# morispi/CONSENT

Measured on AMD Instinct MI355X. Metric: corrected windows/sec, higher is better.
Workload: dtype u8/int16 (2-bit bases, integer DP); 1 GPU; pacbio_d150_msa150: synthetic PacBio-profile piles, 500 bp windows, depth 150, maxMSA 150, k=9, solid=4, commonKMers=8, minAnchors=2; distinct_windows_per_run=704512, engines_per_gpu=4, engines_requested=4, engine_allocation_runs=0, hw_queues=4, overflow_windows=0, template_fallback_windows=0

## Files before the change

### consent_amd/csrc/cw_index.h

```cpp
#ifndef CW_INDEX_H
#define CW_INDEX_H

#include "cw_device.h"

typedef __attribute__((address_space(3))) uint32_t* cw_l32w;
typedef __attribute__((address_space(3))) const uint32_t* cw_l32;
typedef __attribute__((address_space(1))) const uint32_t* cw_g32;
typedef __attribute__((address_space(3))) uint16_t* cw_l16w;
typedef __attribute__((address_space(1))) uint16_t* cw_g16w;
#define CW_IDX_THREADS 1024
#define CW_IDX_WAVES 16
#define CW_IDX_LDS_BYTES 163840
#define CW_TMAX 2048
#define CW_EX_SLOTS 1024
#define CW_EX_BITS 10
#define CW_EXP_SLOTS 8
#define CW_EXG_SLOTS 262144
#define CW_TH_SLOTS 4096
#ifndef CW_IDX_BYTES_MIN_N
#define CW_IDX_BYTES_MIN_N 64u
#endif
#define CW_IDX_STAGE_OFF 139776
#define CW_IDX_STAGE_N 192
#define CW_IDX_STAGE_WORDS ((CW_IDX_LDS_BYTES - CW_IDX_STAGE_OFF - 16 - CW_IDX_STAGE_N * 8) / 4)
// ... 635 lines not shown
    while (xe != 0ull && (uint32_t)(xe >> 32) != key + 1) { slot = (slot + 1) & (CW_EX_SLOTS - 1); xe = ex[slot]; }
    return (uint32_t)xe;
}
__device__ __forceinline__ uint32_t idx_nibble_cand(const uint32_t v, const uint32_t add) {
    return ((((v & 0x0F0F0F0Fu) + add) & 0x10101010u) >> 4) | (((((v >> 4) & 0x0F0F0F0Fu) + add) & 0x10101010u) >> 3);
}
__device__ __forceinline__ bool idx_export_walk(const IdxLds& L, const IdxWin& win, const DevScratch& sc, const cw_params& prm, const uint32_t n_keys, const uint32_t nib_words,
                                                const unsigned long long* exg, const bool big_ex, uint32_t& total, unsigned long long& _pt) {
    const int tid = threadIdx.x;
    const uint32_t* const tab = L.tab();
    const uint32_t keys_per_word = n_keys >= 8 ? 8 : n_keys;
    const uint32_t wpt = (nib_words + CW_IDX_THREADS - 1) / CW_IDX_THREADS;
    const uint32_t w_beg = min(nib_words, (uint32_t)tid * wpt), w_cnt = min(nib_words, w_beg + wpt) - w_beg;
    uint32_t lk[CW_EXP_SLOTS];
    bool wide = false;
    uint32_t mine = 0, n_first = 0xFFFFFFFFu;
    const uint32_t add = (16u - (prm.solid < 15u ? prm.solid : 15u)) * 0x01010101u;
    auto scan_word = [&](const uint32_t v, const uint32_t wd) {
        if (v == 0) return;
        uint32_t cand = idx_nibble_cand(v, add);
        if (keys_per_word < 8) cand &= (1u << (8 * ((keys_per_word + 1) / 2))) - 1u;
        while (cand) {
            const uint32_t bpos = (uint32_t)__ffs((int)cand) - 1u;
            cand &= cand - 1u;
            const uint32_t q = (bpos >> 3) * 2u + (bpos & 1u);
            const uint32_t nib = (v >> (4 * q)) & 15u;
            const uint32_t key = wd * 8 + q;
            uint32_t c = nib;
            if (nib == 15u) c = 15u + idx_ex_lookup(L.ex(), exg, big_ex, key);
            if (c < prm.solid) continue;
#pragma unroll
            for (int z = 0; z < CW_EXP_SLOTS; ++z) if ((uint32_t)z == mine) lk[z] = key | (c << 18);
            wide = wide || c >= (1u << 14);
            mine++;
        }
    };
    if (w_cnt && (w_cnt & 3u) == 0u) {
        const uint32_t nq = w_cnt >> 2, q0 = (uint32_t)tid % nq;
        for (uint32_t i = 0; i < nq; ++i) {
            uint32_t r = i + q0;
            if (r == nq) n_first = mine;
            r = r >= nq ? r - nq : r;
            const uint32_t wd = w_beg + 4u * r;
            const uint4 v4 = *(const uint4*)&tab[wd];
            if ((v4.x | v4.y | v4.z | v4.w) == 0u) continue;
            scan_word(v4.x, wd); scan_word(v4.y, wd + 1u); scan_word(v4.z, wd + 2u); scan_word(v4.w, wd + 3u);
        }
    } else {
        const uint32_t r0 = w_cnt ? (uint32_t)tid % w_cnt : 0u;
        for (uint32_t i = 0; i < w_cnt; ++i) {
            uint32_t r = i + r0;
            if (r == w_cnt) n_first = mine;
            r = r >= w_cnt ? r - w_cnt : r;
            scan_word(tab[w_beg + r], w_beg + r);
        }
    }
    CW_PROF(sc.ctr, CW_PS_IDX_EXPORT_SCAN, tid == 0);
    const uint32_t off = cw_block_exscan(mine, L.scan_tmp(), &total);
    const bool fits = total <= win.solid_cap;
    if (n_first > mine) n_first = mine;
    if (fits && (mine > CW_EXP_SLOTS || wide)) {
        CW_IDX_ROUTE(sc.ctr, true, CW_IR_REWALK);
        uint32_t o = win.solid_base + off;
        for (uint32_t i = 0; i < w_cnt && mine; ++i) {
            const uint32_t wd = w_beg + i;
            const uint32_t v = tab[wd];
            if (v == 0) continue;
            uint32_t cand = idx_nibble_cand(v, add);
            if (keys_per_word < 8) cand &= (1u << (8 * ((keys_per_word + 1) / 2))) - 1u;
            while (cand) {
                const uint32_t bpos = (uint32_t)__ffs((int)cand) - 1u;
                cand &= cand - 1u;
                const uint32_t q = (bpos >> 3) * 2u + (bpos & 1u);
                const uint32_t nib = (v >> (4 * q)) & 15u;
                const uint32_t key = wd * 8 + q;
                uint32_t c = nib;
                if (nib == 15u) c = 15u + idx_ex_lookup(L.ex(), exg, big_ex, key);
                if (c >= prm.solid) { sc.solid_key[o] = key; sc.solid_cnt[o] = c; o++; }
            }
        }
    } else if (fits && mine) {
#pragma unroll
        for (int z = 0; z < CW_EXP_SLOTS; ++z) {
            if ((uint32_t)z < mine) {
                const uint32_t pos = (uint32_t)z < n_first ? (uint32_t)z + (mine - n_first) : (uint32_t)z - n_first;
                sc.solid_key[win.solid_base + off + pos] = lk[z] & 0x3FFFFu;
                sc.solid_cnt[win.solid_base + off + pos] = lk[z] >> 18;
            }
        }
    }
    return fits;
}
__device__ __forceinline__ bool idx_export_nibbles(const IdxLds& L, const IdxWin& win, const DevScratch& sc, const cw_params& prm, const uint32_t n_keys, const uint32_t nib_words,
                                                   const bool big_ex, unsigned long long& _pt) {
    const int tid = threadIdx.x;
    const unsigned long long* const exg = idx_wg_scratch(sc);
    uint32_t total;
    bool fits;
    const uint32_t NI = nib_words >> 12;
    if (prm.solid <= 15u && (nib_words & 4095u) == 0u && NI >= 1u && NI <= 8u) {
        const uint32_t add = (16u - (prm.solid < 15u ? prm.solid : 15u)) * 0x01010101u;
        uint32_t m[8];
        CW_IDX_ROUTE(sc.ctr, tid == 0, CW_IR_EXPORT_MASKS);
        idx_read_masks<8>(L.tab(), NI, m, [&](const uint32_t v) -> uint32_t {
            const uint32_t c = idx_nibble_cand(v, add);
            return (c | (c >> 6) | (c >> 12) | (c >> 18)) & 0xFFu;
        });
        CW_PROF(sc.ctr, CW_PS_IDX_EXPORT_SCAN, tid == 0);
        fits = idx_export_masks<8>(m, L.tab(), NI, 0u, win.solid_base, L.scan_tmp(), sc.solid_key, sc.solid_cnt, total,
            [&](const uint32_t n) -> bool { return n <= win.solid_cap; },
            [&](const uint32_t v, const uint32_t q, const uint32_t key) -> uint32_t {
                uint32_t c = (v >> (4u * q)) & 15u;
                if (c == 15u) c += idx_ex_lookup(L.ex(), exg, big_ex, key);
                return c;
            });
    } else {
        CW_IDX_ROUTE(sc.ctr, tid == 0, CW_IR_EXPORT_WALK);
        fits = idx_export_walk(L, win, sc, prm, n_keys, nib_words, exg, big_ex, total, _pt);
    }
    if (tid == 0) {
        win.wi->n_solid = fits ? total : 0;
        if (!fits) idx_stop(win.wi, sc.ctr, CW_WHY_SOLIDCAP);
    }
    __syncthreads();
    return fits;
}

__device__ __forceinline__ void idx_template_table(const IdxLds& L, const IdxPile& pl, const IdxMatrix& M, const uint32_t k, const uint32_t nk0) {
    const int tid = threadIdx.x;
    uint32_t* const th = L.th(); uint32_t* const tkey = L.tkey();
    if (M.tfit) M.clear_lds(nk0 * M.Np);
    if (tid == 0) { L.misc()[4] = 0; L.misc()[5] = 0; }
    for (uint32_t i = tid; i < CW_TH_SLOTS; i += CW_IDX_THREADS) th[i] = 0;
    for (uint32_t i = tid; i < L.seen_words() * 32u; i += CW_IDX_THREADS) { L.tsup()[i] = 0; L.trep()[i] = 0; L.tcand()[i] = -1; }
    for (uint32_t tp = tid; tp < nk0; tp += CW_IDX_THREADS) tkey[tp] = pl.stw ? cw_kmer_at(pl.s_words, tp, k) : cw_kmer_at(pl.bases + pl.seq_word_off[pl.s0], tp, k);
    __syncthreads();
    for (uint32_t tp = tid; tp < nk0; tp += CW_IDX_THREADS) {
        const uint32_t key = tkey[tp];
        uint32_t bkt = CW_TH_HOME(key);
        for (bool placed = false; !placed; bkt = (bkt + 1) & (CW_TH_BUCKETS - 1)) {
            for (uint32_t j = 0; j < 4u && !placed; ++j) {
                const uint32_t prev = atomicCAS(&th[bkt * 4u + j], 0u, (tp + 1u) | CW_TH_FP(key));
                if (prev == 0) placed = true;
                else if ((prev & ~4095u) == CW_TH_FP(key) && tkey[CW_TH_POS(prev) - 1] == key) { L.trep()[CW_TH_POS(prev) - 1] = 1; placed = true; }
            }
        }
    }
    __syncthreads();
}

#define CW_IDX_HIT_CAP (CW_EXG_SLOTS * 2u)
__device__ __forceinline__ bool idx_hit_list(const IdxMatrix& M, const uint32_t N) { return !M.tfit && N <= 1024u; }

__device__ __forceinline__ void idx_support(const IdxLds& L, const IdxPile& pl, const IdxMatrix& M, const DevScratch& sc, const uint32_t k, const uint32_t kmask) {
    const int lane = threadIdx.x & 63, wave = threadIdx.x >> 6;
    const uint32_t N = pl.N, Np = M.Np;
    uint32_t* const th = L.th(); uint32_t* const tkey = L.tkey(); uint32_t* const tsup = L.tsup(); uint8_t* const trep = L.trep(); uint32_t* const misc = L.misc();
    uint16_t* const P_lds = M.P_lds;
    const bool tfit = M.tfit, hl = idx_hit_list(M, N);
    uint32_t* const hitlist = (uint32_t*)idx_wg_scratch(sc);
    const uint32_t hit_cap = CW_IDX_HIT_CAP;
    const bool fp_exact = k <= 10u;
    auto support_seq = [&](const auto words, const uint32_t len, const uint32_t s, uint32_t* my_seen) {
        const uint32_t nk = len >= k ? len - k + 1 : 0, nwd = (len + 15u) >> 4;
        for (uint32_t p0 = (uint32_t)lane * 4u; p0 < nk; p0 += 256u) {
            uint32_t key4[4], bkt4[4], e1[4];
            idx_keys4(idx_window(words, p0, nwd), k, kmask, key4);
#pragma unroll
            for (uint32_t q = 0; q < 4u; ++q) bkt4[q] = CW_TH_HOME(key4[q]);
            if (fp_exact) {
                auto match = [&](const uint4 v, const uint32_t fp1) -> uint32_t { return min(min(v.x - fp1, v.y - fp1), min(v.z - fp1, v.w - fp1)); };
                uint4 v4[4];
#pragma unroll
                for (uint32_t q = 0; q < 4u; ++q) v4[q] = p0 + q < nk ? *(const uint4*)&th[bkt4[q] * 4u] : make_uint4(0u, 0u, 0u, 0u);
                uint32_t pend = 0;
#pragma unroll
                for (uint32_t q = 0; q < 4u; ++q) { e1[q] = match(v4[q], CW_TH_FP(key4[q]) + 1u); if (e1[q] >= (uint32_t)CW_TMAX && v4[q].w != 0u) pend |= 1u << q; }
                while (__ballot(pend != 0u) != 0ull) {
#pragma unroll
                    for (uint32_t q = 0; q < 4u; ++q) {
                        if ((pend >> q) & 1u) {
                            bkt4[q] = (bkt4[q] + 1u) & (CW_TH_BUCKETS - 1);
                            const uint4 v = *(const uint4*)&th[bkt4[q] * 4u];
                            e1[q] = match(v, CW_TH_FP(key4[q]) + 1u);
                            if (e1[q] < (uint32_t)CW_TMAX || v.w == 0u) pend &= ~(1u << q);
                        }
                    }
                }
            } else {
#pragma unroll
                for (uint32_t q = 0; q < 4u; ++q) e1[q] = p0 + q < nk ? (uint32_t)cw_tpl_lookup(th, tkey, key4[q]) : 0xFFFFFFFFu;
            }
            uint32_t old4[4];
#pragma unroll
            for (uint32_t q = 0; q < 4u; ++q) {
                const uint32_t e = e1[q];
                old4[q] = e < (uint32_t)CW_TMAX ? atomicOr(&my_seen[e >> 5], 1u << (e & 31u)) : 0u;
            }
            uint32_t n_list = 0, my_list = 0;
#pragma unroll
            for (uint32_t q = 0; q < 4u; ++q) {
                const uint32_t e = e1[q], p = p0 + q;
                const bool hit = e < (uint32_t)CW_TMAX;
                if (hit) {
                    if (old4[q] & (1u << (e & 31u))) trep[e] = 1;
                    else atomicAdd(&tsup[e], 1u);
                    if (tfit) P_lds[__umul24(e, Np) + s] = (uint16_t)p;
                    else if (hl && p >= 2048u) misc[5] = 1;
                }
                if (!tfit && hl) {
                    const unsigned long long hm = __ballot(hit && p < 2048u);
                    if (hit && p < 2048u) my_list |= (n_list + (uint32_t)__popcll(hm & ((1ull << lane) - 1ull))) << (8u * q);
                    n_list += (uint32_t)__popcll(hm);
                }
            }
            if (!tfit && hl && n_list) {
                uint32_t base = 0;
                if (lane == 0) base = atomicAdd(&misc[4], n_list);
                base = (uint32_t)cw_lane_value((int)base, 0);
#pragma unroll
                for (uint32_t q = 0; q < 4u; ++q) {
                    const uint32_t p = p0 + q, hi_ = base + ((my_list >> (8u * q)) & 255u);
                    if (e1[q] < (uint32_t)CW_TMAX && p < 2048u && hi_ < hit_cap) hitlist[hi_] = (e1[q] << 21) | (s << 11) | p;
                }
            }
        }
    };
    for (uint32_t s = wave; s < N; s += CW_IDX_WAVES) {
        uint32_t* my_seen = L.seen() + wave * L.seen_words();
        if ((uint32_t)lane < L.seen_words()) my_seen[lane] = 0;
        cw_wave_sync();
        idx_with_seq(pl, s, [&](const auto words, const uint32_t len) { support_seq(words, len, s, my_seen); });
        cw_wave_sync();
    }
    __syncthreads();
}

__device__ __forceinline__ uint32_t idx_candidates(const IdxLds& L, const uint32_t nk0, const int sup_min) {
    const int tid = threadIdx.x;
    uint32_t A = 0;
    for (uint32_t tb = 0; tb < nk0; tb += CW_IDX_THREADS) {
        const uint32_t tp = tb + (uint32_t)tid;
        uint32_t ok = 0;
        if (tp < nk0) {
            const int rep = cw_tpl_lookup(L.th(), L.tkey(), L.tkey()[tp]);
            ok = (rep == (int)tp && L.trep()[tp] == 0 && (int)L.tsup()[tp] >= sup_min) ? 1u : 0u;
        }
        uint32_t a_round;
        const uint32_t off = A + cw_block_exscan(ok, L.scan_tmp(), &a_round);
        if (ok) { L.tcand()[tp] = (int16_t)off; L.cand_tp()[off] = (uint16_t)tp; }
        A += a_round;
        __syncthreads();
    }
    __syncthreads();
    return A;
}

__device__ __forceinline__ bool idx_fill_matrix(const IdxLds& L, const IdxPile& pl, const IdxWin& win, const IdxMatrix& M, const DevScratch& sc, const uint32_t k, const uint32_t kmask,
                                                const uint32_t A) {
    const int tid = threadIdx.x, wave = tid >> 6;
    const uint32_t N = pl.N, Np = M.Np;
    if (M.pg && (uint64_t)A * Np > sc.p_fallback_elems) {
        if (tid == 0) { idx_stop(win.wi, sc.ctr, CW_WHY_MATRIX); win.wi->arena_used = (uint64_t)A * Np > 0xFFFFFFFFull ? 0xFFFFFFFFu : A * Np; }
        __builtin_amdgcn_wave_barrier();
        return false;
    }
    const uint32_t* const hitlist = (const uint32_t*)idx_wg_scratch(sc);
    const uint32_t n_hits = L.misc()[4];
    const bool from_list = idx_hit_list(M, N) && n_hits <= CW_IDX_HIT_CAP && L.misc()[5] == 0u;
    if (!M.tfit) {
        if (!M.pg) M.clear_lds(A * Np);
        else for (uint32_t i = tid; i < A * Np; i += CW_IDX_THREADS) M.wr(i, CW_NONE16);
        __builtin_amdgcn_fence(__ATOMIC_RELEASE, "workgroup");
        __syncthreads();
        __builtin_amdgcn_fence(__ATOMIC_ACQUIRE, "workgroup");
        if (from_list) {
            for (uint32_t i0 = tid; i0 < n_hits; i0 += 4u * CW_IDX_THREADS) {
                uint32_t h4[4];
#pragma unroll
                for (uint32_t u = 0; u < 4u; ++u) { const uint32_t i = i0 + u * CW_IDX_THREADS; h4[u] = i < n_hits ? hitlist[i] : 0xFFFFFFFFu; }
#pragma unroll
                for (uint32_t u = 0; u < 4u; ++u) {
                    const uint32_t h = h4[u];
                    const int a = i0 + u * CW_IDX_THREADS < n_hits ? L.tcand()[h >> 21] : -1;
                    if (a >= 0) M.wr((uint32_t)a * Np + ((h >> 11) & 1023u), h & 2047u);
                }
            }
        } else
        for (uint32_t s = wave; s < N; s += CW_IDX_WAVES) {
            idx_pile_seq<IDX_WAVE>(pl, s, k, kmask, [&](const uint32_t, const uint32_t p, const uint32_t key, const uint32_t) {
                const int e = cw_tpl_lookup(L.th(), L.tkey(), key);
                if (e < 0) return;
                const int a = L.tcand()[e];
                if (a >= 0) M.wr((uint32_t)a * Np + s, p);
            });
        }
        __syncthreads();
    }
    return true;
}

struct IdxPres {
    uint8_t* clean;
    uint8_t* didx;
    unsigned long long* pres;
    uint16_t* dirty;
    unsigned long long* badm;
    uint8_t* rowid;
    uint16_t* rowanc;
    bool use_bits, has_bm, has_delta;
    uint32_t n_rows;
    uint32_t W;
    uint32_t n_dirty;
};
__device__ __forceinline__ IdxPres idx_presence_carve(const IdxLds& L, const IdxMatrix& M, const uint32_t A, const uint32_t N, const uint32_t nk0) {
    uint8_t* const lds = L.lds;
    const uint32_t Nw = (N + 63u) >> 6;
    IdxPres ps;
    ps.clean = (uint8_t*)L.seen();
    ps.didx = ps.clean + 1024;
    ps.pres = (unsigned long long*)(M.P_lds + (M.pg ? 0 : (((size_t)(M.tfit ? nk0 : A) * M.Np + 3u) & ~(size_t)3u)));
    ps.dirty = (uint16_t*)(ps.pres + (size_t)A * Nw);
    ps.badm = (unsigned long long*)(lds + (((size_t)((uint8_t*)(ps.dirty + N) - lds) + 7u) & ~(size_t)7u));
    ps.use_bits = N <= 2048u && ((uint8_t*)(ps.dirty + N) <= lds + CW_IDX_STAGE_OFF);
    ps.has_bm = false; ps.has_delta = false;
    ps.n_rows = 0;
    ps.W = 1;
    ps.rowid = (uint8_t*)(ps.badm + (size_t)A * 4);
    ps.rowanc = (uint16_t*)(lds + (((size_t)(ps.rowid + A - lds) + 1u) & ~(size_t)1u));
    ps.n_dirty = 0;
    return ps;
}

__device__ __forceinline__ IdxPres idx_classify_sequences(const IdxLds& L, const IdxWin& win, const IdxMatrix& M, IdxPres ps, const DevScratch& sc, const uint32_t A, unsigned long long& _pt) {
    const int tid = threadIdx.x, lane = tid & 63, wave = tid >> 6;
    const uint32_t N = win.N, Np = M.Np;
    uint8_t* const lds = L.lds; uint32_t* const misc = L.misc();
    uint8_t* const clean = ps.clean; uint16_t* const dirty = ps.dirty; unsigned long long* const badm = ps.badm;
    uint32_t W = 1;
    auto scan_seq = [&](const uint32_t s, const bool fwd, const bool mark, const uint32_t d) -> uint32_t {
        int run = -1;
        uint32_t n_bad = 0;
        for (uint32_t a0 = 0; a0 < A; a0 += 64) {
            const uint32_t ai = a0 + lane;
            const uint32_t a = fwd ? ai : A - 1u - ai;
            const uint32_t pv = ai < A ? M.rd(M.row(a) * Np + s) : (uint32_t)CW_NONE16;
            const int v = pv != CW_NONE16 ? (fwd ? (int)pv : (int)(0xFFFEu - pv)) : -1;
            const int inc = cw_wave_scan_max(v);
            int before = cw_wave_shr1(inc, -1);
            before = max(before, run);
            const bool bad = v >= 0 && v <= before;
            if (mark) { if (bad) atomicOr(&badm[(size_t)a * W + (d >> 6)], 1ull << (d & 63u)); }
            else n_bad += (uint32_t)__popcll(__ballot(bad));
            run = max(run, cw_lane_value(inc, 63));
        }
        return n_bad;
    };
    for (uint32_t s = wave; s < N; s += CW_IDX_WAVES) {
        const uint32_t nf = scan_seq(s, true, false, 0);
        uint32_t c = 1;
        if (nf) c = scan_seq(s, false, false, 0) < nf ? 2u : 0u;
        if (lane == 0) clean[s] = (uint8_t)c;
    }
    if (tid == 0) misc[3] = 0;
    __syncthreads();
    CW_PROF(sc.ctr, CW_PS_IDX_CLEAN, tid == 0);
    for (uint32_t s = tid; s < N; s += CW_IDX_THREADS)
        if (clean[s] != 1) dirty[atomicAdd(&misc[3], 1u)] = (uint16_t)s;
    __syncthreads();
    const uint32_t nd = misc[3];
    W = (nd + 63u) >> 6;
    if (W == 0u) W = 1u;
    const bool masks = nd > 0 && nd <= 255u  && W <= (N <= 1024u ? 4u : 1u) && (uint8_t*)(ps.rowanc + CW_AB_ROWS_MAX) <= lds + CW_IDX_STAGE_OFF;
    if (masks) {
        for (uint32_t i = tid; i < A * W; i += CW_IDX_THREADS) badm[i] = 0ull;
        __syncthreads();
        for (uint32_t d = wave; d < nd; d += CW_IDX_WAVES) { const uint32_t s = dirty[d]; scan_seq(s, clean[s] == 0, true, d); }
        __syncthreads();
        uint32_t ok2[2] = {0u, 0u}, off2[2] = {0u, 0u};
        uint32_t n_rows = 0;
#pragma nounroll
        for (uint32_t r2 = 0; r2 < 2u; ++r2) {
            const uint32_t an = r2 * CW_IDX_THREADS + (uint32_t)tid;
            if (r2 * CW_IDX_THREADS >= A) break;
            if (an < A) for (uint32_t x = 0; x < W; ++x) ok2[r2] |= badm[(size_t)an * W + x] != 0ull ? 1u : 0u;
            uint32_t n_round;
            off2[r2] = n_rows + cw_block_exscan(ok2[r2], misc + 16, &n_round);
            n_rows += n_round;
            __syncthreads();
        }
        ps.has_delta = n_rows >= 1u && n_rows <= CW_AB_ROWS_MAX && cw_ab_bytes(A, N, nd, n_rows) <= ((uint64_t)win.ab_cap << 4);
        ps.has_bm = W == 1u || ps.has_delta;
        if (ps.has_delta) {
            for (uint32_t r2 = 0; r2 < 2u; ++r2) {
                const uint32_t an = r2 * CW_IDX_THREADS + (uint32_t)tid;
                if (an < A) ps.rowid[an] = ok2[r2] ? (uint8_t)off2[r2] : (uint8_t)0xFF;
                if (ok2[r2]) ps.rowanc[off2[r2]] = (uint16_t)an;
            }
        } else n_rows = 0;
        ps.n_rows = n_rows;
        if (ps.has_bm && (uint32_t)tid < nd) { const uint32_t s = dirty[tid]; clean[s] = (uint8_t)0x80u; if (N <= 1024u) ps.didx[s] = (uint8_t)tid; else clean[s] = (uint8_t)(0x80u | (uint32_t)tid); }
        __syncthreads();
    }
    ps.W = W;
    return ps;
}

__device__ __forceinline__ void idx_presence(const IdxMatrix& M, const IdxPres& ps, const uint32_t A, const uint32_t N) {
    const int lane = threadIdx.x & 63, wave = threadIdx.x >> 6;
    const uint32_t Np = M.Np, Nw = (N + 63u) >> 6, W = ps.W;
    for (uint32_t w = 0; w < Nw; ++w) {
        const uint32_t s = w * 64 + lane;
        const uint32_t c = s < N ? (uint32_t)ps.clean[s] : 0u;
        const bool plain = c == 1u, part = ps.has_bm && (c & 0x80u) != 0u;
        const uint32_t d = part ? (N <= 1024u ? (uint32_t)ps.didx[s] : (c & 63u)) : 0u;
        for (uint32_t a = wave; a < A; a += CW_IDX_WAVES) {
            bool good = plain;
            if (part) good = !((ps.badm[(size_t)a * W + (d >> 6)] >> (d & 63u)) & 1ull);
            const bool on = s < N && M.rd(M.row(a) * Np + s) != CW_NONE16 && good;
            const unsigned long long bal = __ballot(on);
            if (lane == 0) ps.pres[(size_t)a * Nw + w] = bal;
        }
    }
    __syncthreads();
}

__device__ __forceinline__ bool idx_hand_over(const IdxLds& L, const IdxWin& win, const IdxMatrix& M, const IdxPres& ps, const DevScratch& sc, const uint32_t A) {
    const int tid = threadIdx.x, lane = tid & 63, wave = tid >> 6;
    const uint32_t N = win.N, Np = M.Np, Nw = (N + 63u) >> 6, W = ps.W, n_dirty = ps.n_dirty, n_rows = ps.n_rows;
    const unsigned long long* const badm = ps.badm; const uint16_t* const dirty = ps.dirty;
    if (cw_ab_bytes(A, N, n_dirty, n_rows) > ((uint64_t)win.ab_cap << 4)) {
        if (tid == 0) { idx_stop(win.wi, sc.ctr, CW_WHY_MATRIX); win.wi->arena_used = 0xFFFFFFFFu; }
        __builtin_amdgcn_wave_barrier();
        return false;
    }
    const CwAbCarve<uint8_t*> ab = cw_ab_carve(sc.ablock + ((size_t)win.ab_base << 4), A, N, n_dirty, n_rows);
    uint32_t* hdr = (uint32_t*)ab.hdr; uint32_t* ckey = (uint32_t*)ab.ckey; unsigned long long* gpres = (unsigned long long*)ab.pres; uint16_t* gdirty = (uint16_t*)ab.dirty;
    unsigned long long* gbadm = (unsigned long long*)ab.badm;
    const uint32_t Ap = cw_ab_ap(A);
    if (tid == 0) { hdr[0] = A; hdr[1] = N; hdr[2] = n_dirty; hdr[3] = (ps.use_bits ? 1u : 0u) | (ps.has_bm && W == 1u ? 2u : 0u) | (ps.has_delta ? 4u : 0u); hdr[4] = n_rows; }
    for (uint32_t a = tid; a < A; a += CW_IDX_THREADS) ckey[a] = L.tkey()[L.cand_tp()[a]];
    if (ps.use_bits) {
        for (uint32_t i = tid; i < A * Nw; i += CW_IDX_THREADS) gpres[i] = ps.pres[i];
        for (uint32_t i = tid; i < n_dirty; i += CW_IDX_THREADS) gdirty[i] = dirty[i];
        if (ps.has_bm && W == 1u) for (uint32_t a = tid; a < A; a += CW_IDX_THREADS) gbadm[a] = badm[a];
        if (ps.has_delta) {
            for (uint32_t a = tid; a < A; a += CW_IDX_THREADS) ab.rowid[a] = ps.rowid[a];
            for (uint32_t r = wave; r < n_rows; r += CW_IDX_WAVES) {
                const uint32_t x = ps.rowanc[r];
                for (uint32_t y0 = 0; y0 < Ap; y0 += 64) {
                    const uint32_t y = y0 + lane;
                    uint32_t cnt = 0;
                    if (y < A && y != x) {
                        for (uint32_t wd = 0; wd < W; ++wd) {
                            const unsigned long long bmx = badm[(size_t)x * W + wd], bmy = badm[(size_t)y * W + wd];
                            unsigned long long mm = y < x ? bmx & ~bmy : bmx;
                            while (mm) {
                                const uint32_t d = wd * 64u + (uint32_t)__ffsll((long long)mm) - 1u;
                                mm &= mm - 1ull;
                                const uint32_t sd = dirty[d];
                                const uint32_t px = M.rd(M.row(x) * Np + sd), py = M.rd(M.row(y) * Np + sd);
                                cnt += y > x ? ((px < py && py != CW_NONE16) ? 1u : 0u) : (py < px ? 1u : 0u);
                            }
                        }
                    }
                    if (y < Ap) ab.delta[(size_t)r * Ap + y] = (uint8_t)cnt;
                }
            }
        }
    }
    {
        const uint32_t* src = (const uint32_t*)(M.pg ? M.P_glb : M.P_lds);
        uint32_t* dst = (uint32_t*)ab.P;
        const uint32_t half = Np >> 1;
        if (M.tfit) {
            for (uint32_t a = wave; a < A; a += CW_IDX_WAVES)
                for (uint32_t j = lane; j < half; j += 64) dst[a * half + j] = src[(uint32_t)L.cand_tp()[a] * half + j];
        } else {
            const uint32_t n2 = A * half;
            if (!M.pg) {
                const uint32_t n4 = n2 >> 2;
                for (uint32_t i = tid; i < n4; i += CW_IDX_THREADS) ((uint4*)dst)[i] = ((const uint4*)src)[i];
                for (uint32_t i = (n4 << 2) + tid; i < n2; i += CW_IDX_THREADS) dst[i] = src[i];
            } else
            for (uint32_t i = tid; i < n2; i += CW_IDX_THREADS) dst[i] = src[i];
        }
    }
    return true;
}

__global__ void __launch_bounds__(CW_IDX_THREADS) cw_index_kernel(DevBatch b, DevScratch sc, cw_params prm) {
    extern __shared__ __attribute__((aligned(16))) uint8_t lds[];
    const int tid = threadIdx.x;
    const uint32_t k = prm.k;
    const bool direct = k <= 9;
    const uint32_t n_keys = direct ? 1u << (2 * k) : 0u;
    const uint32_t kmask = k >= 16u ? 0xFFFFFFFFu : (1u << (2u * k)) - 1u;
    const uint32_t nib_words = direct ? (n_keys >= 8 ? n_keys / 8 : 1) : 0u;
    IdxLds L;
    L.lds = lds; L.wide = false;

    for (;;) {
        __syncthreads();
        if (tid == 0) { L.st_hdr()[1] = atomicAdd(&sc.ctr->next_window, 1u); L.st_hdr()[0] = 0; }
        __syncthreads();
        const uint32_t w = L.st_hdr()[1];
        if (w >= b.n_windows) break;
        WinInfo* wi = &sc.win[w];
        if (wi->status == CW_WIN_OVERFLOW) continue;
        const uint32_t s0 = b.win_first_seq[w];
        const IdxWin win(wi);
        const uint32_t N = win.N, L0 = win.L0;
        L.wide = L0 >= k && L0 - k + 1u > 1024u;
        const IdxPile pl = idx_stage_pile(b, L, s0, N);
        CW_IDX_ROUTE(sc.ctr, tid == 0, (pl.stw ? CW_IR_STAGED : 0u) | (L.wide ? CW_IR_WIDE : 0u));
        CW_PROF_T0();
        if (!direct) {
            if (!idx_count_hashed(L, pl, win, sc, prm, kmask)) continue;
        } else {
            bool done8, big_ex;
            if (!idx_count_bytes(L, pl, win, sc, prm, kmask, n_keys, done8, _pt)) continue;
            CW_IDX_ROUTE(sc.ctr, tid == 0, done8 ? CW_IR_BYTES_DONE : CW_IR_NIBBLES);
            if (!done8) {
                if (!idx_count_nibbles(L, pl, win, sc, prm, kmask, nib_words, big_ex, _pt)) continue;
                CW_IDX_ROUTE(sc.ctr, tid == 0 && big_ex, CW_IR_BIG_EX);
                if (!idx_export_nibbles(L, win, sc, prm, n_keys, nib_words, big_ex, _pt)) continue;
            }
        }
        CW_PROF(sc.ctr, CW_PS_IDX_EXPORT, tid == 0);
        const uint32_t nk0 = L0 >= k ? L0 - k + 1 : 0;
        const int sup_min = min((int)prm.common_kmers, (int)N / 2);
        if (nk0 == 0 || nk0 > CW_TMAX) {
            if (tid == 0) {
                if (nk0 == 0) wi->status = CW_WIN_TEMPLATE;
                else idx_stop(wi, sc.ctr, CW_WHY_TEMPLATE);
            }
            __builtin_amdgcn_wave_barrier();
            continue;
        }
        IdxMatrix M;
        M.P_lds = L.P(); M.P_glb = sc.p_fallback + (size_t)blockIdx.x * sc.p_fallback_elems; M.cand_tp = L.cand_tp();
        M.Np = cw_ab_np(N);
        M.pg = false;
        M.tfit = idx_matrix_need(nk0, N, M.Np) <= (uint64_t)L.p_cap() * 2;
        idx_template_table(L, pl, M, k, nk0);
        CW_PROF(sc.ctr, CW_PS_IDX_TPLHASH, tid == 0);
        idx_support(L, pl, M, sc, k, kmask);
        CW_PROF(sc.ctr, CW_PS_IDX_SUPPORT, tid == 0);
        const uint32_t A = idx_candidates(L, nk0, sup_min);
        CW_PROF(sc.ctr, CW_PS_IDX_CAND, tid == 0);
        M.pg = !M.tfit && idx_matrix_need(A, N, M.Np) > (uint64_t)L.p_cap() * 2;
        CW_IDX_ROUTE(sc.ctr, tid == 0, (M.tfit ? CW_IR_TFIT : 0u) | (M.pg ? CW_IR_PG : 0u) | (idx_hit_list(M, N) ? CW_IR_HIT_LIST : 0u));
        if (!idx_fill_matrix(L, pl, win, M, sc, k, kmask, A)) continue;
        CW_PROF(sc.ctr, CW_PS_IDX_PFILL, tid == 0);
        IdxPres ps = idx_presence_carve(L, M, A, N, nk0);
        CW_IDX_ROUTE(sc.ctr, tid == 0 && ps.use_bits, CW_IR_USE_BITS);
        if (ps.use_bits) {
            ps = idx_classify_sequences(L, win, M, ps, sc, A, _pt);
            CW_PROF(sc.ctr, CW_PS_IDX_DIRTY, tid == 0);
            idx_presence(M, ps, A, N);
            ps.n_dirty = L.misc()[3];
        }
        CW_PROF(sc.ctr, CW_PS_IDX_PRESENCE, tid == 0);
        if (!idx_hand_over(L, win, M, ps, sc, A)) continue;
        CW_PROF(sc.ctr, CW_PS_IDX_HANDOVER, tid == 0);
    }
}

#endif
```

Baseline: 297,000 windows/s.

## Replace per-sequence wave scans with column-sweep classification and fused presence pass

```diff
diff --git a/consent_amd/csrc/cw_index.h b/consent_amd/csrc/cw_index.h
--- a/consent_amd/csrc/cw_index.h
+++ b/consent_amd/csrc/cw_index.h
@@ -961,7 +961,6 @@
 
 struct IdxPres {
     uint8_t* clean;
-    uint8_t* didx;
     unsigned long long* pres;
     uint16_t* dirty;
     unsigned long long* badm;
@@ -977,7 +976,6 @@
     const uint32_t Nw = (N + 63u) >> 6;
     IdxPres ps;
     ps.clean = (uint8_t*)L.seen();
-    ps.didx = ps.clean + 1024;
     ps.pres = (unsigned long long*)(M.P_lds + (M.pg ? 0 : (((size_t)(M.tfit ? nk0 : A) * M.Np + 3u) & ~(size_t)3u)));
     ps.dirty = (uint16_t*)(ps.pres + (size_t)A * Nw);
     ps.badm = (unsigned long long*)(lds + (((size_t)((uint8_t*)(ps.dirty + N) - lds) + 7u) & ~(size_t)7u));
@@ -991,51 +989,185 @@
     return ps;
 }
 
+#define CW_IDX_SW_ITEMS 32u
+static_assert(2u * CW_IDX_SW_ITEMS * 64u * 4u <= CW_TH_SLOTS * 4u, "records and counts of every item fit the template table");
+struct IdxSweep {
+    uint32_t T, C, len;
+    uint32_t* rec;
+    uint32_t* cnt;
+    uint16_t* dix;
+};
+__device__ __forceinline__ IdxSweep idx_sweep_plan(const IdxLds& L, const uint32_t A, const uint32_t N) {
+    IdxSweep sw;
+    sw.T = (N + 63u) >> 6;
+    sw.C = sw.T >= CW_IDX_WAVES ? 1u : CW_IDX_WAVES / sw.T;
+    sw.len = (A + sw.C - 1u) / sw.C;
+    sw.rec = L.th(); sw.cnt = sw.rec + CW_IDX_SW_ITEMS * 64u; sw.dix = (uint16_t*)sw.cnt;
+    return sw;
+}
+__device__ __forceinline__ uint32_t idx_sweep_wave() { return (uint32_t)__builtin_amdgcn_readfirstlane((int)(threadIdx.x >> 6)); }
+struct IdxItem { uint32_t t, c, a_lo, a_hi, s; bool valid; };
+__device__ __forceinline__ IdxItem idx_sweep_item(const IdxSweep& sw, const uint32_t item, const uint32_t A, const uint32_t N) {
+    IdxItem it;
+    it.t = item / sw.C; it.c = item - it.t * sw.C;
+    it.a_lo = min(it.c * sw.len, A); it.a_hi = min(it.a_lo + sw.len, A);
+    it.s = it.t * 64u + (threadIdx.x & 63u); it.valid = it.s < N;
+    return it;
+}
+template <bool TFIT, typename PT> struct IdxCol {
+    PT P; const __attribute__((address_space(3))) uint16_t* cand_tp; uint32_t Np, s;
+    __device__ __forceinline__ IdxCol(PT P_, const IdxMatrix& M, const IdxItem& it, const uint32_t N)
+        : P(P_), cand_tp((const __attribute__((address_space(3))) uint16_t*)M.cand_tp), Np(M.Np), s(min(it.s, N - 1u)) {}
+    __device__ __forceinline__ uint32_t at(const uint32_t a) const { return (uint32_t)P[(TFIT ? (uint32_t)cand_tp[a] : a) * Np + s]; }
+};
+__device__ __forceinline__ void idx_sweep_incoming(const IdxSweep& sw, const IdxItem& it, uint32_t& in_mx, uint32_t& in_mn) {
+    in_mx = 0u; in_mn = CW_NONE16;
+    const uint32_t* const r = sw.rec + it.t * sw.C * 64u + (threadIdx.x & 63u);
+    for (uint32_t c2 = 0; c2 < it.c; ++c2) in_mx = max(in_mx, r[c2 * 64u] & 0xFFFFu);
+    for (uint32_t c2 = it.c + 1u; c2 < sw.C; ++c2) in_mn = min(in_mn, r[c2 * 64u] >> 16);
+}
+template <bool TFIT, typename PT> __device__ __forceinline__ void idx_sweep_records(const PT P, const IdxMatrix& M, const IdxSweep& sw, const uint32_t A, const uint32_t N) {
+    const uint32_t lane = threadIdx.x & 63u, wave = idx_sweep_wave();
+    for (uint32_t item = wave; item < sw.T * sw.C; item += CW_IDX_WAVES) {
+        const IdxItem it = idx_sweep_item(sw, item, A, N);
+        const IdxCol<TFIT, PT> col(P, M, it, N);
+        uint32_t mx = 0u, mn = CW_NONE16;
+        if (it.a_lo < it.a_hi) {
+            const uint32_t last = it.a_hi - 1u;
+            for (uint32_t a = it.a_lo; a < it.a_hi; a += 4u) {
+                uint32_t pv[4];
+#pragma unroll
+                for (uint32_t u = 0; u < 4u; ++u) pv[u] = col.at(min(a + u, last));
+#pragma unroll
+                for (uint32_t u = 0; u < 4u; ++u) { mx = max(mx, (pv[u] + 1u) & 0xFFFFu); mn = min(mn, pv[u]); }
+            }
+        }
+        sw.rec[item * 64u + lane] = mx | (mn << 16);
+    }
+}
+template <bool TFIT, typename PT> __device__ __forceinline__ void idx_sweep_counts(const PT P, const IdxMatrix& M, const IdxSweep& sw, const uint32_t A, const uint32_t N) {
+    const uint32_t lane = threadIdx.x & 63u, wave = idx_sweep_wave();
+    for (uint32_t item = wave; item < sw.T * sw.C; item += CW_IDX_WAVES) {
+        const IdxItem it = idx_sweep_item(sw, item, A, N);
+        const IdxCol<TFIT, PT> col(P, M, it, N);
+        uint32_t runf, runb, nf = 0u, nb = 0u;
+        idx_sweep_incoming(sw, it, runf, runb);
+        if (it.a_lo < it.a_hi) {
+            const uint32_t n = it.a_hi - it.a_lo, last = it.a_hi - 1u;
+            for (uint32_t i = 0; i < n; i += 2u) {
+                uint32_t pf[2], pb[2];
+#pragma unroll
+                for (uint32_t u = 0; u < 2u; ++u) { const uint32_t iu = min(i + u, n - 1u); pf[u] = col.at(it.a_lo + iu); pb[u] = col.at(last - iu); }
+#pragma unroll
+                for (uint32_t u = 0; u < 2u; ++u) {
+                    if (i + u < n) {
+                        nf += pf[u] < runf ? 1u : 0u; runf = max(runf, (pf[u] + 1u) & 0xFFFFu);
+                        nb += pb[u] != CW_NONE16 && pb[u] >= runb ? 1u : 0u; runb = min(runb, pb[u]);
+                    }
+                }
+            }
+        }
+        sw.cnt[item * 64u + lane] = it.valid ? nf | (nb << 16) : 0u;
+    }
+}
+template <bool TFIT, typename PT> __device__ __forceinline__ void idx_sweep_presence(const PT P, const IdxMatrix& M, const IdxSweep& sw, const IdxPres& ps, const uint32_t A, const uint32_t N,
+                                                                                      const uint32_t W, const bool masks) {
+    const uint32_t lane = threadIdx.x & 63u, wave = idx_sweep_wave(), Nw = sw.T;
+    unsigned long long* const pres = ps.pres; unsigned long long* const badm = ps.badm;
+    for (uint32_t item = wave; item < sw.T * sw.C; item += CW_IDX_WAVES) {
+        const IdxItem it = idx_sweep_item(sw, item, A, N);
+        if (it.a_lo >= it.a_hi) continue;
+        const IdxCol<TFIT, PT> col(P, M, it, N);
+        const uint32_t cls = it.valid ? (uint32_t)ps.clean[it.s] : 3u;
+        const bool fdirty = masks && cls == 0u, bdirty = masks && cls == 2u;
+        const unsigned long long m_plain = __ballot(cls == 1u), m_f = __ballot(fdirty), m_b = __ballot(bdirty);
+        const uint32_t d = fdirty || bdirty ? (uint32_t)sw.dix[it.s] : 0u;
+        const unsigned long long dbit = 1ull << (d & 63u);
+        uint32_t runf = 0u, runb = CW_NONE16;
+        if (masks) idx_sweep_incoming(sw, it, runf, runb);
+        const uint32_t last = it.a_hi - 1u;
+        for (uint32_t a = it.a_lo; a < it.a_hi; a += 4u) {
+            uint32_t pv[4];
+#pragma unroll
+            for (uint32_t u = 0; u < 4u; ++u) pv[u] = col.at(min(a + u, last));
+#pragma unroll
+            for (uint32_t u = 0; u < 4u; ++u) {
+                if (a + u < it.a_hi) {
+                    const bool bad = pv[u] < runf;
+                    runf = max(runf, (pv[u] + 1u) & 0xFFFFu);
+                    const unsigned long long here = __ballot(pv[u] != CW_NONE16), badw = __ballot(bad) & m_f;
+                    if (badw != 0ull) { if (bad && fdirty) atomicOr(&badm[(a + u) * W + (d >> 6)], dbit); }
+                    const unsigned long long word = here & (m_plain | (m_f & ~badw));
+                    if (lane == 0u) pres[(a + u) * Nw + it.t] = word;
+                }
+            }
+        }
+        if (m_b != 0ull) {
+            for (uint32_t a = it.a_hi; a-- > it.a_lo;) {
+                const uint32_t p = col.at(a);
+                const bool bad = p != CW_NONE16 && p >= runb;
+                runb = min(runb, p);
+                if (bdirty && bad) atomicOr(&badm[a * W + (d >> 6)], dbit);
+                const unsigned long long word = __ballot(p != CW_NONE16 && !bad) & m_b;
+                if (lane == 0u && word != 0ull) pres[a * Nw + it.t] |= word;
+            }
+        }
+    }
+}
+#define CW_IDX_SWEEP(fn, ...)                                                     \
+    do {                                                                          \
+        if (M.pg) fn<false>((cw_g16w)M.P_glb, __VA_ARGS__);                       \
+        else if (M.tfit) fn<true>((cw_l16w)M.P_lds, __VA_ARGS__);                 \
+        else fn<false>((cw_l16w)M.P_lds, __VA_ARGS__);                            \
+    } while (0)
+
 __device__ __forceinline__ IdxPres idx_classify_sequences(const IdxLds& L, const IdxWin& win, const IdxMatrix& M, IdxPres ps, const DevScratch& sc, const uint32_t A, unsigned long long& _pt) {
-    const int tid = threadIdx.x, lane = tid & 63, wave = tid >> 6;
-    const uint32_t N = win.N, Np = M.Np;
+    const int tid = threadIdx.x;
+    const uint32_t N = win.N;
     uint8_t* const lds = L.lds; uint32_t* const misc = L.misc();
     uint8_t* const clean = ps.clean; uint16_t* const dirty = ps.dirty; unsigned long long* const badm = ps.badm;
-    uint32_t W = 1;
-    auto scan_seq = [&](const uint32_t s, const bool fwd, const bool mark, const uint32_t d) -> uint32_t {
-        int run = -1;
-        uint32_t n_bad = 0;
-        for (uint32_t a0 = 0; a0 < A; a0 += 64) {
-            const uint32_t ai = a0 + lane;
-            const uint32_t a = fwd ? ai : A - 1u - ai;
-            const uint32_t pv = ai < A ? M.rd(M.row(a) * Np + s) : (uint32_t)CW_NONE16;
-            const int v = pv != CW_NONE16 ? (fwd ? (int)pv : (int)(0xFFFEu - pv)) : -1;
-            const int inc = cw_wave_scan_max(v);
-            int before = cw_wave_shr1(inc, -1);
-            before = max(before, run);
-            const bool bad = v >= 0 && v <= before;
-            if (mark) { if (bad) atomicOr(&badm[(size_t)a * W + (d >> 6)], 1ull << (d & 63u)); }
-            else n_bad += (uint32_t)__popcll(__ballot(bad));
-            run = max(run, cw_lane_value(inc, 63));
-        }
-        return n_bad;
-    };
-    for (uint32_t s = wave; s < N; s += CW_IDX_WAVES) {
-        const uint32_t nf = scan_seq(s, true, false, 0);
-        uint32_t c = 1;
-        if (nf) c = scan_seq(s, false, false, 0) < nf ? 2u : 0u;
-        if (lane == 0) clean[s] = (uint8_t)c;
-    }
-    if (tid == 0) misc[3] = 0;
-    __syncthreads();
+    const IdxSweep sw = idx_sweep_plan(L, A, N);
+    if (sw.C > 1u) {
+        CW_IDX_SWEEP(idx_sweep_records, M, sw, A, N);
+        __syncthreads();
+    }
+    CW_IDX_SWEEP(idx_sweep_counts, M, sw, A, N);
+    __syncthreads();
+    for (uint32_t s = tid; s < N; s += CW_IDX_THREADS) {
+        {
+            const uint32_t* const c = sw.cnt + (s >> 6) * sw.C * 64u + (s & 63u);
+            uint32_t nf = 0u, nb = 0u;
+            for (uint32_t c2 = 0; c2 < sw.C; ++c2) { const uint32_t v = c[c2 * 64u]; nf += v & 0xFFFFu; nb += v >> 16; }
+            const uint32_t cls = nf == 0u ? 1u : nb < nf ? 2u : 0u;
+            clean[s] = (uint8_t)cls;
+        }
+    }
     CW_PROF(sc.ctr, CW_PS_IDX_CLEAN, tid == 0);
-    for (uint32_t s = tid; s < N; s += CW_IDX_THREADS)
-        if (clean[s] != 1) dirty[atomicAdd(&misc[3], 1u)] = (uint16_t)s;
-    __syncthreads();
-    const uint32_t nd = misc[3];
-    W = (nd + 63u) >> 6;
+    uint32_t nd = 0;
+#pragma nounroll
+    for (uint32_t r2 = 0; r2 < 2u; ++r2) {
+        if (r2 * CW_IDX_THREADS >= N) break;
+        const uint32_t s = r2 * CW_IDX_THREADS + (uint32_t)tid;
+        const uint32_t isd = s < N && clean[s] != 1u ? 1u : 0u;
+        uint32_t n_round;
+        const uint32_t off = nd + cw_block_exscan(isd, misc + 16, &n_round);
+        if (isd) { dirty[off] = (uint16_t)s; sw.dix[s] = (uint16_t)off; }
+        nd += n_round;
+        __syncthreads();
+    }
+    ps.n_dirty = nd;
+    uint32_t W = (nd + 63u) >> 6;
     if (W == 0u) W = 1u;
     const bool masks = nd > 0 && nd <= 255u  && W <= (N <= 1024u ? 4u : 1u) && (uint8_t*)(ps.rowanc + CW_AB_ROWS_MAX) <= lds + CW_IDX_STAGE_OFF;
     if (masks) {
         for (uint32_t i = tid; i < A * W; i += CW_IDX_THREADS) badm[i] = 0ull;
         __syncthreads();
-        for (uint32_t d = wave; d < nd; d += CW_IDX_WAVES) { const uint32_t s = dirty[d]; scan_seq(s, clean[s] == 0, true, d); }
-        __syncthreads();
+    }
+    CW_PROF(sc.ctr, CW_PS_IDX_DIRTY, tid == 0);
+    CW_IDX_SWEEP(idx_sweep_presence, M, sw, ps, A, N, W, masks);
+    __syncthreads();
+    CW_PROF(sc.ctr, CW_PS_IDX_PRESENCE, tid == 0);
+    if (masks) {
         uint32_t ok2[2] = {0u, 0u}, off2[2] = {0u, 0u};
         uint32_t n_rows = 0;
 #pragma nounroll
@@ -1058,30 +1190,20 @@
             }
         } else n_rows = 0;
         ps.n_rows = n_rows;
-        if (ps.has_bm && (uint32_t)tid < nd) { const uint32_t s = dirty[tid]; clean[s] = (uint8_t)0x80u; if (N <= 1024u) ps.didx[s] = (uint8_t)tid; else clean[s] = (uint8_t)(0x80u | (uint32_t)tid); }
+        if (!ps.has_bm) {
+            unsigned long long* const dm = (unsigned long long*)sw.rec;
+            for (uint32_t t = (uint32_t)tid >> 6; t < sw.T; t += CW_IDX_WAVES) {
+                const uint32_t s = t * 64u + ((uint32_t)tid & 63u);
+                const unsigned long long m = __ballot(s < N && clean[s] != 1u);
+                if ((tid & 63) == 0) dm[t] = m;
+            }
+            __syncthreads();
+            for (uint32_t i = tid; i < A * sw.T; i += CW_IDX_THREADS) ps.pres[i] &= ~dm[i % sw.T];
+        }
         __syncthreads();
     }
     ps.W = W;
     return ps;
-}
-
-__device__ __forceinline__ void idx_presence(const IdxMatrix& M, const IdxPres& ps, const uint32_t A, const uint32_t N) {
-    const int lane = threadIdx.x & 63, wave = threadIdx.x >> 6;
-    const uint32_t Np = M.Np, Nw = (N + 63u) >> 6, W = ps.W;
-    for (uint32_t w = 0; w < Nw; ++w) {
-        const uint32_t s = w * 64 + lane;
-        const uint32_t c = s < N ? (uint32_t)ps.clean[s] : 0u;
-        const bool plain = c == 1u, part = ps.has_bm && (c & 0x80u) != 0u;
-        const uint32_t d = part ? (N <= 1024u ? (uint32_t)ps.didx[s] : (c & 63u)) : 0u;
-        for (uint32_t a = wave; a < A; a += CW_IDX_WAVES) {
-            bool good = plain;
-            if (part) good = !((ps.badm[(size_t)a * W + (d >> 6)] >> (d & 63u)) & 1ull);
-            const bool on = s < N && M.rd(M.row(a) * Np + s) != CW_NONE16 && good;
-            const unsigned long long bal = __ballot(on);
-            if (lane == 0) ps.pres[(size_t)a * Nw + w] = bal;
-        }
-    }
-    __syncthreads();
 }
 
 __device__ __forceinline__ bool idx_hand_over(const IdxLds& L, const IdxWin& win, const IdxMatrix& M, const IdxPres& ps, const DevScratch& sc, const uint32_t A) {
@@ -1217,10 +1339,7 @@
         if (ps.use_bits) {
             ps = idx_classify_sequences(L, win, M, ps, sc, A, _pt);
             CW_PROF(sc.ctr, CW_PS_IDX_DIRTY, tid == 0);
-            idx_presence(M, ps, A, N);
-            ps.n_dirty = L.misc()[3];
-        }
-        CW_PROF(sc.ctr, CW_PS_IDX_PRESENCE, tid == 0);
+        }
         if (!idx_hand_over(L, win, M, ps, sc, A)) continue;
         CW_PROF(sc.ctr, CW_PS_IDX_HANDOVER, tid == 0);
     }
```

Result: no change. 297,000 windows/s (-0.0%).
